# ipo-lab/lqp_py

Measured on AMD Instinct MI355X. Metric: QPs/sec forward+backward, batch=128 dz=500 tol=1e-5, higher is better.
Workload: dtype f32; 1 GPU; BASELINE configs[2]: batch=128/GPU dz=500 m=1 box+equality QP, ADMM forward + fixed-point backward, eps 1e-5, scale+adaptive_rho defaults; global_batch=128, seeds=10 batches, seeds 0..9 per rank, cycled, iters=60, checks=4, launch_mode=3, sync=False, linsolve=spd, loop_workgroups_per_qp=2, parallelism=batch-sharded x1, rccl_world_size=1

## Files before the change

lqp_py_amd/csrc/lqp_boxqp.hpp:

```cpp
#pragma once
#include <type_traits>
#include "lqp_common.hpp"
#include "lqp_lu.hpp"
#include "lqp_lu_big.hpp"
#include "lqp_lu2.hpp"
#include "lqp_lu_wide.hpp"
#include "lqp_trsv.hpp"
#include "lqp_spd.hpp"

namespace lqp {

enum { ST_DONE = 0, ST_FINAL_ITER = 1, ST_GATE = 2, ST_NFACTOR = 3, ST_RHO_UPDATED = 4,
       ST_TIMEOUT = 5, ST_NCHECK = 6, ST_NOTSPD = 7,
       ST_VOTE = 8,
       ST_ANY_LB = 12, ST_ANY_UB = 13,
       ST_RESUME = 14,
       ST_WORDS = 16 };
enum { RP_LB = 1, RP_UB = 2, RP_TIMEOUT = 4, RP_NOTSPD = 8 };
enum { CT_NOTOPT = 0, CT_ARRIVE = 1, CT_WANTS = 2, CT_TRIG = 3, CT_WORDS = 4 };
template <typename T>
__device__ __forceinline__ void trace_check(unsigned int* __restrict__ vtrace, const int it, const int check_solved, const int ring,
                                            const T pri, const T dua) {
    if (!vtrace) return;
    const int c = it / check_solved;
// ... 2351 lines not shown
        if (lane == 0) wtot[w] = __popcll(bal);
        __syncthreads();
        int base = nf;
#pragma unroll
        for (int ww = 0; ww < LQP_NW; ++ww) {
            const int c = wtot[ww];
            if (ww < w) base += c;
            nf += c;
        }
        if (keep) {
            fl[base + before] = i;
            if (blockIdx.y == 0) P.fidx[(size_t)b * n + base + before] = i;
        }
    }
    if (tid == 0 && blockIdx.y == 0) P.nred[b] = nf + m;
    __syncthreads();
    const int wy = blockIdx.y, ny = gridDim.y;
    constexpr int GQ = 8;
    for (int a0 = (w * ny + wy) * 2; a0 < nf; a0 += LQP_NW * ny * 2) {
        const int a1 = a0 + 1 < nf ? a0 + 1 : a0;
        const int i0 = fl[a0], i1 = fl[a1];
        const T* q0 = Q + (size_t)i0 * n;
        const T* q1 = Q + (size_t)i1 * n;
        const T dg0 = P.kkt ? kkt_weight(P, b, i0) : T(1e-8), dg1 = P.kkt ? kkt_weight(P, b, i1) : T(1e-8);
        for (int c0 = 0; c0 < nf; c0 += 64 * GQ) {
            T v0[GQ], v1[GQ];
#pragma unroll
            for (int q = 0; q < GQ; ++q) {
                const int c = c0 + lane + 64 * q;
                const int col = fl[c < nf ? c : nf - 1];
                v0[q] = q0[col];
                v1[q] = q1[col];
            }
#pragma unroll
            for (int q = 0; q < GQ; ++q) {
                const int c = c0 + lane + 64 * q;
                if (c < nf) {
                    M[(size_t)a0 * Np + c] = c == a0 ? v0[q] + dg0 : v0[q];
                    if (a1 != a0) M[(size_t)a1 * Np + c] = c == a1 ? v1[q] + dg1 : v1[q];
                }
            }
        }
        for (int r = lane; r < m; r += 64) {
            M[(size_t)a0 * Np + nf + r] = A[(size_t)r * n + i0];
            if (a1 != a0) M[(size_t)a1 * Np + nf + r] = A[(size_t)r * n + i1];
        }
        if (lane == 0 && P.g) { rhs[a0] = -g[i0]; if (a1 != a0) rhs[a1] = -g[i1]; }
    }
    for (int r = w * ny + wy; r < m; r += LQP_NW * ny) {
        T* mr = M + (size_t)(nf + r) * Np;
        for (int c = lane; c < nf; c += 64) mr[c] = A[(size_t)r * n + fl[c]];
        for (int c = lane; c < m; c += 64) mr[nf + c] = (c == r && !P.kkt) ? T(1e-8) : T(0);
        if (lane == 0) rhs[nf + r] = T(0);
    }
}

__device__ __forceinline__ float bwd_equil_scale(const float d) {
    if (!(d > 0.f) || !(d < 3.0e38f)) return 1.f;
    const int h = (int)((__float_as_uint(d) >> 23) & 0xFFu) - 127;
    return __uint_as_float((unsigned int)(127 - (h >> 1)) << 23);
}
template <int LQP_ANY = 0>
__global__ __launch_bounds__(LQP_NT) void k_bwd_build_chol(const BwdParams<float> P) {
    extern __shared__ __attribute__((aligned(32))) char smem[];
    const int b = blockIdx.x, n = P.n, m = P.m, Np = P.Np;
    const int tid = threadIdx.x, lane = tid & 63, w = tid >> 6;
    int* fl = (int*)smem;
    int* wtot = fl + round_up(n, 8);
    const float* x = P.x + (size_t)b * n;
    const float* u = P.u + (size_t)b * n;
    const float* lb = P.lb + (size_t)b * n;
    const float* ub = P.ub + (size_t)b * n;
    const float* g = P.g + (size_t)b * n;
    const float* Q = P.Q + (size_t)b * n * n;
    const float* A = P.A ? P.A + (size_t)b * m * n : nullptr;
    const int Kmax = round_up(n, LQP_NB) / LQP_NB, Npm = Kmax * LQP_NB;
    float* Ls = P.packed + (size_t)b * sym_blocks(Kmax) * LQP_BLK;
    float* AF = P.M + (size_t)b * Np * Np;
    float* rhs = P.rhs + (size_t)b * Np;
    if (tid == 0 && blockIdx.y == 0) P.info[b] = 0;
    float* wl = (float*)(wtot + LQP_NW + 8);
    bool keep = false;
    if (tid < n) {
        if (P.kkt) { keep = true; wl[tid] = kkt_weight(P, b, tid); }
        else {
            const float sxu = x[tid] + u[tid];
            keep = !(sxu > ub[tid] || sxu < lb[tid]);
        }
    }
    const unsigned long long bal = __ballot(keep);
    const int before = __popcll(bal & ((1ull << lane) - 1ull));
    if (lane == 0) wtot[w] = __popcll(bal);
    __syncthreads();
    int base = 0, nf = 0;
#pragma unroll
    for (int ww = 0; ww < LQP_NW; ++ww) {
        const int c = wtot[ww];
        if (ww < w) base += c;
        nf += c;
    }
    if (keep) {
        fl[base + before] = tid;
        if (blockIdx.y == 0) P.fidx[(size_t)b * n + base + before] = tid;
    }
    if (tid == 0 && blockIdx.y == 0) P.nred[b] = nf + m;
    __syncthreads();
    const int Kb = round_up(nf, LQP_NB) / LQP_NB;
    const int r = tid >> 4, c4 = (tid & 15) * 4;
    const int nblk = sym_blocks(Kb);
    float* const sl = wl + round_up(n, 8);
    for (int a = tid; a < Npm; a += LQP_NT) {
        float sv = 1.f;
        if (P.bsc && a < nf) sv = bwd_equil_scale(Q[(size_t)fl[a] * n + fl[a]] + (P.kkt ? wl[fl[a]] : 1e-8f));
        sl[a] = sv;
        if (P.bsc && blockIdx.y == 0) P.bsc[(size_t)b * Np + a] = sv;
    }
    __syncthreads();
    for (int t = blockIdx.y; t < nblk; t += gridDim.y) {
        int j = 0;
        while (sym_idx(j + 1, j + 1, Kb) <= t && j + 1 < Kb) ++j;
        const int i = j + (t - sym_idx(j, j, Kb));
        const int a = i * 64 + r;
        const bool rok = a < nf;
        const size_t rowoff = (size_t)fl[rok ? a : 0] * n;
        float q4[4];
#pragma unroll
        for (int e = 0; e < 4; ++e) {
            const int c = j * 64 + c4 + e;
            q4[e] = Q[rowoff + fl[c < nf ? c : 0]];
        }
        V4<float> v;
#pragma unroll
        for (int e = 0; e < 4; ++e) {
            const int c = j * 64 + c4 + e;
            float val = (a == c) ? 1.f : 0.f;
            if (rok && c < nf) val = ((q4[e] + (a == c ? (P.kkt ? wl[fl[a]] : 1e-8f) : 0.f)) * sl[a]) * sl[c];
            v.v[e] = val;
        }
        *(V4<float>*)(Ls + (size_t)t * LQP_BLK + tid * 4) = v;
    }
    if (blockIdx.y == 0) {
        if (P.phase != 1)
            for (int a = tid; a < Npm; a += LQP_NT) rhs[a] = a < nf ? -g[fl[a]] * sl[a] : 0.f;
        for (int q = 0; q < m; ++q)
            for (int a = tid; a < Npm; a += LQP_NT) AF[(size_t)q * Npm + a] = a < nf ? A[(size_t)q * n + fl[a]] * sl[a] : 0.f;
    }
}

__host__ __device__ inline int bwd_chol_lds_bytes(int n, int m, int nr = 2) {
    const int Kmax = round_up(n, LQP_NB) / LQP_NB, Npm = Kmax * LQP_NB;
    const int a0 = spd_lds_bytes(Kmax > SPD_MAXK ? SPD_MAXK : Kmax);
    const int a = (Kmax < SPD_MAXK && chol_la_lds_bytes(Kmax) > a0) ? chol_la_lds_bytes(Kmax) : a0;
    const int c = ((1 + nr + m) * Npm + nr * 64 + nr * LQP_NW * 64 + m * m + 2 * m + 8) * 4;
    return a > c ? a : c;
}
template <int NRV = 0, bool F16 = false>
__global__ __launch_bounds__(LQP_NT) void k_bwd_chol_solve(const BwdParams<float> P) {
    extern __shared__ __attribute__((aligned(32))) char smem[];
    const int b = blockIdx.x, n = P.n, m = P.m, Np = P.Np;
    const int tid = threadIdx.x, lane = tid & 63, w = tid >> 6;
    const int Kmax = round_up(n, LQP_NB) / LQP_NB, Npm = Kmax * LQP_NB;
    const int nf = P.nred[b] - m;
    const int Kb = round_up(nf, LQP_NB) / LQP_NB, Nb = Kb * LQP_NB;
    float* Ls = P.packed + (size_t)b * sym_blocks(Kmax) * LQP_BLK;
    const float* AF = P.M + (size_t)b * Np * Np;
    float* rhs = P.rhs + (size_t)b * Np;
    unsigned long long dt0 = P.dbg ? clock64() : 0;
    if (Kb > 0 && P.phase != 2) {
        if (Kb <= P.la_maxk) wg_chol_factor_la<F16>(Ls, Kb, P.info + b, smem, P.dbg ? P.dbg + (size_t)b * 8 : nullptr);
        else if (Kb <= SPD_MAXK) wg_chol_factor(Ls, Kb, P.info + b, smem);
        else wg_chol_factor_big(Ls, Kb, P.info + b, smem);
    }
    if (P.host_report && (P.early_report || P.phase == 1) && !P.reported) {
        __syncthreads();
        if (tid == 0)
            __hip_atomic_store(P.host_report + b, __hip_atomic_load(P.info + b, __ATOMIC_RELAXED, __HIP_MEMORY_SCOPE_AGENT),
                               __ATOMIC_RELAXED, __HIP_MEMORY_SCOPE_SYSTEM);
    }
    if (P.phase == 1) return;
    __syncthreads();
    if (P.dbg && tid == 0) { const unsigned long long t = clock64(); P.dbg[(size_t)b * 8 + 0] = t - dt0; dt0 = t; P.dbg[(size_t)b * 8 + 3] = Kb; }
    constexpr int NR = NRV == 4 ? 4 : 2;
    float* acc = (float*)smem;
    float* u0 = acc + (size_t)NR * Npm;
    float* G = u0 + Npm;
    float* t = G + (size_t)m * Npm;
    float* part = t + NR * 64;
    float* S = part + NR * LQP_NW * 64;
    float* wv = S + m * m;
    float* dn = wv + m;
    if (P.phase == 2) {
        const float* g = P.g + (size_t)b * n;
        const int* fidx = P.fidx + (size_t)b * n;
        const float* bs_ = P.bsc ? P.bsc + (size_t)b * Np : nullptr;
        for (int e = tid; e < Nb; e += LQP_NT) u0[e] = e < nf ? -g[fidx[e]] * (bs_ ? bs_[e] : 1.f) : 0.f;
    } else {
        for (int e = tid; e < Nb; e += LQP_NT) u0[e] = rhs[e];
    }
    for (int q = 0; q < m; ++q)
        for (int e = tid; e < Nb; e += LQP_NT) G[(size_t)q * Npm + e] = AF[(size_t)q * Npm + e];
    __syncthreads();
    if (Kb > 0)
        for (int c0 = 0; c0 < 1 + m; c0 += NR)
            wg_chol_solve_n<NR>(Ls, Kb, u0 + (size_t)c0 * Npm, Npm, (1 + m - c0) < NR ? (1 + m - c0) : NR, acc, t, part,
                                (P.dbg && P.la_maxk == 0) ? P.dbg + (size_t)b * 8 : nullptr);
    if (P.dbg && tid == 0) { const unsigned long long t = clock64(); P.dbg[(size_t)b * 8 + 1] = t - dt0; dt0 = t; }
    if (m > 0) {
        for (int e = w; e < m * m + m; e += LQP_NW) {
            const int q = e < m * m ? e / m : e - m * m;
            const float* rv = e < m * m ? G + (size_t)(e - q * m) * Npm : u0;
            float a = 0.f;
            for (int i = lane; i < nf; i += 64) a += AF[(size_t)q * Npm + i] * rv[i];
            a = wave_sum(a);
            if (lane == 0) {
                if (e < m * m) S[e] = a - ((e / m == e % m) ? 1e-8f : 0.f);
                else wv[q] = a;
            }
        }
        __syncthreads();
        {
            const int rr = tid / (m + 1), jj = tid - rr * (m + 1);
            const bool mine = tid < m * (m + 1);
            int* pivrow = (int*)dn;
            for (int c = 0; c < m; ++c) {
                if (tid == 0) {
                    int pr = c;
                    float best = tabs(S[c * m + c]);
                    for (int r2 = c + 1; r2 < m; ++r2) if (tabs(S[r2 * m + c]) > best) { best = tabs(S[r2 * m + c]); pr = r2; }
                    const bool skip = !(best > 0.f);
                    if (skip && P.info[b] == 0) P.info[b] = nf + c + 1;
                    pivrow[0] = pr; pivrow[1] = skip ? 1 : 0;
                }
                __syncthreads();
                const int pr = pivrow[0];
                const bool skip = pivrow[1] != 0;
                float* const rowc = jj < m ? S + c * m + jj : wv + c;
                float* const rowp = jj < m ? S + pr * m + jj : wv + pr;
                float* const rowr = jj < m ? S + rr * m + jj : wv + rr;
                if (!skip && pr != c && tid <= m) {
                    const float tmp = *rowc; *rowc = *rowp; *rowp = tmp;
                }
                __syncthreads();
                const float inv = skip ? 0.f : 1.f / S[c * m + c];
                const float f = (mine && !skip) ? S[rr * m + c] : 0.f;
                __syncthreads();
                if (!skip && tid <= m) *rowc *= inv;
                __syncthreads();
                if (mine && !skip && rr != c) *rowr -= f * *rowc;
                __syncthreads();
            }
            for (int q = tid; q < m; q += LQP_NT) dn[q] = wv[q];
        }
        __syncthreads();
    }
    for (int a = tid; a < nf; a += LQP_NT) {
        float d = u0[a];
        for (int q = 0; q < m; ++q) d -= G[(size_t)q * Npm + a] * dn[q];
        rhs[a] = P.bsc ? d * P.bsc[(size_t)b * Np + a] : d;
    }
    for (int q = tid; q < m; q += LQP_NT) rhs[nf + q] = dn[q];
    if (P.dbg && tid == 0) P.dbg[(size_t)b * 8 + 2] = clock64() - dt0;
}

template <typename T>
__global__ __launch_bounds__(LQP_NT) void k_bwd_residual(const BwdParams<T> P) {
    extern __shared__ __attribute__((aligned(32))) char smem[];
    const int b = blockIdx.x, n = P.n, m = P.m, Np = P.Np;
    const int tid = threadIdx.x, lane = tid & 63, w = tid >> 6;
    T* dvf = (T*)smem;
    T* dn = dvf + round_up(n, 8);
    int* fl = (int*)(dn + round_up(m > 0 ? m : 1, 8));
    const int nf = P.nred[b] - m;
    const T* d = P.rhs + (size_t)b * Np;
    T* r = P.rhs2 + (size_t)b * Np;
    const T* Q = P.Q + (size_t)b * n * n;
    const T* A = P.A ? P.A + (size_t)b * m * n : nullptr;
    const T* g = P.g + (size_t)b * n;
    for (int i = tid; i < n; i += LQP_NT) dvf[i] = T(0);
    for (int a = tid; a < nf; a += LQP_NT) fl[a] = P.fidx[(size_t)b * n + a];
    for (int q = tid; q < m; q += LQP_NT) dn[q] = d[nf + q];
    __syncthreads();
    for (int a = tid; a < nf; a += LQP_NT) dvf[fl[a]] = d[a];
    __syncthreads();
    constexpr int RG = 4;
    const int ny = (int)gridDim.y, me = (int)blockIdx.y;
    for (int a0 = (w * ny + me) * RG; a0 < nf + m; a0 += LQP_NW * ny * RG) {
        const T* row[RG];
        double acc[RG];
#pragma unroll
        for (int u = 0; u < RG; ++u) {
            const int a = min(a0 + u, nf + m - 1);
            row[u] = a >= nf ? A + (size_t)(a - nf) * n : Q + (size_t)fl[a] * n;
            acc[u] = 0.0;
        }
        for (int j = lane; j < n; j += 64) {
            const double dj = (double)dvf[j];
            T v[RG];
#pragma unroll
            for (int u = 0; u < RG; ++u) v[u] = row[u][j];
#pragma unroll
            for (int u = 0; u < RG; ++u) acc[u] += (double)v[u] * dj;
        }
#pragma unroll
        for (int u = 0; u < RG; ++u) acc[u] = wave_sum(acc[u]);
        if (lane < RG && a0 + lane < nf + m) {
            const int a = a0 + lane;
            double mine = readlane_t(acc[0], 0);
#pragma unroll
            for (int u = 1; u < RG; ++u) { const double t = readlane_t(acc[u], 0); mine = lane == u ? t : mine; }
            double res;
            if (a < nf) {
                const int i = fl[a];
                res = -(double)g[i] - mine - 1e-8 * (double)d[a];
                for (int q = 0; q < m; ++q) res -= (double)A[(size_t)q * n + i] * (double)dn[q];
            } else {
                res = -mine - 1e-8 * (double)dn[a - nf];
            }
            r[a] = (T)res;
        }
    }
    if (me == 0)
        for (int a = nf + m + tid; a < Np; a += LQP_NT) r[a] = T(0);
}

template <typename T> __host__ __device__ inline int solve_lds_bytes(int Np) { return (Np + 64) * (int)sizeof(T) + Np * 4; }

template <typename T>
__global__ __launch_bounds__(LQP_NT) void k_packed_solve(const T* __restrict__ packed_all, const int Nuni, const int Npmax,
                                                         const int Kmax, const int* __restrict__ dest_all,
                                                         T* __restrict__ rhs_all, const int nrhs,
                                                         const size_t rhs_bstride, const int rhs_rstride,
                                                         const int rhs_cstride, const int* __restrict__ Nvec) {
    extern __shared__ __attribute__((aligned(32))) char smem[];
    const int b = blockIdx.x, tid = threadIdx.x;
    const int N = Nvec ? Nvec[b] : Nuni;
    const int K = round_up(N, LQP_NB) / LQP_NB, Np = K * LQP_NB;
    T* v = (T*)smem;
    T* tmp = v + Npmax;
    int* dest = (int*)(tmp + 64);
    const T* packed = packed_all + (size_t)b * packed_blocks(Kmax) * LQP_BLK;
    const int S = K * (K + 1);
    const bool cyclic = true;
    BlockStream<T, LQP_NT> st;
    stream_prime(st, packed, S);
    for (int i = tid; i < Np; i += LQP_NT) dest[i] = dest_all[(size_t)b * Npmax + i];
    __syncthreads();
    T* rhs = rhs_all + (size_t)b * rhs_bstride;
    for (int c = 0; c < nrhs; ++c) {
        for (int i = tid; i < Np; i += LQP_NT) v[dest[i]] = (i < N) ? rhs[(size_t)i * rhs_rstride + (size_t)c * rhs_cstride] : T(0);
        wg_barrier_lds();
        wg_packed_solve(st, packed, K, v, tmp, cyclic && (c + 1 < nrhs));
        if (!cyclic && c + 1 < nrhs) stream_prime(st, packed, S);
        for (int i = tid; i < N; i += LQP_NT) rhs[(size_t)i * rhs_rstride + (size_t)c * rhs_cstride] = v[i];
        __syncthreads();
    }
}

template <typename T>
__global__ __launch_bounds__(LQP_NT) void k_bwd_epilogue(const BwdParams<T> P) {
    extern __shared__ __attribute__((aligned(32))) char smem[];
    const int b = blockIdx.x, n = P.n, m = P.m, Np = P.Np;
    const int tid = threadIdx.x, lane = tid & 63, w = tid >> 6;
    T* dv = (T*)smem;
    T* xs = dv + n;
    T* dnu = xs + n;
    const T rho = (P.rho_mode == 2) ? P.rho_in[b] : P.rho_value;
    const T* d = P.rhs + (size_t)b * Np;
    const T* x = P.x + (size_t)b * n;
    const T poison = P.info[b] != 0 ? T(__builtin_nanf("")) : T(0);
    if (P.host_report && !(P.chol && P.early_report) && !P.lu_reported && tid == 0 && blockIdx.y == 0)
        __hip_atomic_store(P.host_report + b, P.info[b], __ATOMIC_RELAXED, __HIP_MEMORY_SCOPE_SYSTEM);
    if (P.reduced) {
        const int nf = P.nred[b] - m;
        const int* fl = P.fidx + (size_t)b * n;
        const T* d2 = P.rhs2 + (size_t)b * Np;
        for (int i = tid; i < n; i += LQP_NT) { dv[i] = poison; xs[i] = x[i]; }
        __syncthreads();
        for (int a = tid; a < nf; a += LQP_NT) dv[fl[a]] = d[a] + (P.refine ? d2[a] : T(0)) + poison;
        for (int r = tid; r < m; r += LQP_NT) dnu[r] = d[nf + r] + (P.refine ? d2[nf + r] : T(0)) + poison;
    } else {
        for (int i = tid; i < n; i += LQP_NT) { dv[i] = d[i] + poison; xs[i] = x[i]; }
        for (int r = tid; r < m; r += LQP_NT) dnu[r] = d[n + r] + poison;
    }
    __syncthreads();
    const bool first = blockIdx.y == 0;
    if (P.dp && first) for (int i = tid; i < n; i += LQP_NT) P.dp[(size_t)b * n + i] = dv[i];
    if (P.db && first) for (int r = tid; r < m; r += LQP_NT) P.db[(size_t)b * m + r] = -dnu[r];
    if (P.dA && m > 0 && first) {
        const T* nus = P.nus + (size_t)b * m;
        for (int t = tid; t < m * n; t += LQP_NT) {
            const int r = t / n, j = t - r * n;
            P.dA[(size_t)b * m * n + t] = dnu[r] * xs[j] + nus[r] * dv[j];
        }
    }
    const T* Q = P.Q + (size_t)b * n * n;
    const T* A = P.A ? P.A + (size_t)b * m * n : nullptr;
    if (P.kkt && first) {
        for (int i = tid; i < n; i += LQP_NT) {
            const T xi = xs[i];
            const T slo = tmax(xi - P.lb[(size_t)b * n + i], T(1e-8)), shi = tmax(P.ub[(size_t)b * n + i] - xi, T(1e-8));
            const T llo = tmax(P.lams[(size_t)b * 2 * n + i], T(1e-8)), lhi = tmax(P.lams[(size_t)b * 2 * n + n + i], T(1e-8));
            if (P.dlb) P.dlb[(size_t)b * n + i] = llo * (-dv[i] / slo);
            if (P.dub) P.dub[(size_t)b * n + i] = -lhi * (dv[i] / shi);
        }
    }
    const bool need_kkt = (P.dlb || P.dub) && !P.kkt;
    T* dQ = P.dQ ? P.dQ + (size_t)b * n * n : nullptr;
    const bool vec = (n % 4 == 0) && n <= 1024 && dQ && ((((uintptr_t)dQ) % sizeof(V4<T>)) == 0);
    V4<T> xj[4], hj[4];
    if (vec) {
// ... 136 lines not shown
```

lqp_py_amd/csrc/lqp_spd.hpp:

```cpp
#pragma once
#include "lqp_common.hpp"
#include "lqp_lu.hpp"
#include "lqp_trsv.hpp"
#include "lqp_f16x2.hpp"

namespace lqp {

constexpr int SPD_LS = 68;
constexpr int SPD_MAXK = 8;
constexpr int SPD_MAXM = 16;

__host__ __device__ constexpr int sym_blocks(int K) { return K * (K + 1) / 2; }
__host__ __device__ constexpr int sym_idx(int i, int j, int K) { return j * K - j * (j - 1) / 2 + (i - j); }
#ifndef LQP_PIV_WAVES
#define LQP_PIV_WAVES 16
#endif
#ifndef LQP_PIV_WAVES_RS
#define LQP_PIV_WAVES_RS 8
#endif
#ifndef LQP_PIV_NB
#define LQP_PIV_NB 4
#endif
constexpr int PIV_NB = LQP_PIV_NB;
constexpr int PIV_LDS = 2 * PIV_NB * 64 + 64;
// ... 2500 lines not shown
                int si = 0;
                while ((si + 1) * (si + 2) / 2 <= p) ++si;
                const int sj = p - si * (si + 1) / 2;
                if (si == sj && qi == 0 && qj == 1) continue;
                float* T0 = Hs + (size_t)sym_idx(k + 1 + si, k + 1 + sj, K) * LQP_BLK;
                float* C = T0 + (32 * qi) * 64 + 32 * qj + li;
                f32x16 cur;
#pragma unroll
                for (int q = 0; q < 16; ++q) cur[q] = C[quad_row(q, lh) * 64];
                const f32x16 acc = spd_quadrant(Y + ((size_t)si * 64 + 32 * qi) * SPD_LS,
                                                Y + ((size_t)sj * 64 + 32 * qj) * SPD_LS);
                cur -= acc;
#pragma unroll
                for (int q = 0; q < 16; ++q) C[quad_row(q, lh) * 64] = cur[q];
                if (si == sj && qi == 1 && qj == 0) {
#pragma unroll
                    for (int q = 0; q < 16; ++q) T0[li * 64 + 32 + quad_row(q, lh)] = cur[q];
                }
            }
        }
        __syncthreads();
    }
    if (tid == 0 && flag[0] != 0 && *info == 0) *info = flag[0];
}

__device__ __forceinline__ void wg_chol_factor_big(float* __restrict__ Hs, const int K, int* __restrict__ info, char* smem) {
    constexpr int CH = SPD_MAXK - 1;
    const int tid = threadIdx.x, lane = tid & 63, w = tid >> 6;
    const int r = tid >> 4, cq = tid & 15, li = lane & 31, lh = lane >> 5;
    float* Y = (float*)smem;
    float* W = Y + (size_t)CH * 64 * SPD_LS;
    float* WT = W + 64 * SPD_LS;
    float* pcol = WT + 64 * SPD_LS;
    int* flag = (int*)(pcol + PIV_LDS);
    if (tid == 0) flag[0] = 0;
    for (int k = 0; k < K; ++k) {
        const int np = K - 1 - k;
        wg_pivot<LQP_PIV_WAVES>(Hs + (size_t)sym_idx(k, k, K) * LQP_BLK, W, WT, pcol, flag, k * 64);
        __syncthreads();
        *(V4<float>*)(Hs + (size_t)sym_idx(k, k, K) * LQP_BLK + tid * 4) = *(const V4<float>*)(W + r * SPD_LS + cq * 4);
        for (int c0 = 0; c0 < np; c0 += CH) {
            const int cn = (np - c0) < CH ? (np - c0) : CH;
            for (int u = 0; u < cn; ++u)
                *(V4<float>*)(Y + ((size_t)u * 64 + r) * SPD_LS + cq * 4) =
                    *(const V4<float>*)(Hs + (size_t)sym_idx(k + 1 + c0 + u, k, K) * LQP_BLK + tid * 4);
            __syncthreads();
            {
                const int ntask = cn * 4;
                f32x16 acc[2];
#pragma unroll
                for (int u = 0; u < 2; ++u) {
                    const int task = __builtin_amdgcn_readfirstlane(w + 16 * u);
                    if (task < ntask) {
                        const int sl = task >> 2, qi = (task >> 1) & 1, qj = task & 1;
                        const float* Xp = Y + ((size_t)sl * 64 + 32 * qi) * SPD_LS;
                        acc[u] = qj == 0 ? spd_quadrant<1, false>(Xp, W) : spd_quadrant(Xp, W + 32 * SPD_LS);
                    }
                }
                __syncthreads();
#pragma unroll
                for (int u = 0; u < 2; ++u) {
                    const int task = __builtin_amdgcn_readfirstlane(w + 16 * u);
                    if (task < ntask) {
                        const int sl = task >> 2, qi = (task >> 1) & 1, qj = task & 1;
                        float* dst = Y + ((size_t)sl * 64 + 32 * qi) * SPD_LS + 32 * qj + li;
#pragma unroll
                        for (int q = 0; q < 16; ++q) dst[quad_row(q, lh) * SPD_LS] = acc[u][q];
                    }
                }
                __syncthreads();
            }
            for (int u = 0; u < cn; ++u)
                *(V4<float>*)(Hs + (size_t)sym_idx(k + 1 + c0 + u, k, K) * LQP_BLK + tid * 4) =
                    *(const V4<float>*)(Y + ((size_t)u * 64 + r) * SPD_LS + cq * 4);
            __syncthreads();
        }
        __threadfence_block();
        __syncthreads();
        const int ng = (np + BIG_G - 1) / BIG_G;
        for (int ga = 0; ga < ng; ++ga) {
            for (int gb = 0; gb <= ga; ++gb) {
                const int a0 = BIG_G * ga, b0 = BIG_G * gb;
                const int an = (np - a0) < BIG_G ? (np - a0) : BIG_G, bn = (np - b0) < BIG_G ? (np - b0) : BIG_G;
                const int boff = gb == ga ? 0 : BIG_G;
                for (int u = 0; u < an; ++u)
                    *(V4<float>*)(Y + ((size_t)u * 64 + r) * SPD_LS + cq * 4) =
                        *(const V4<float>*)(Hs + (size_t)sym_idx(k + 1 + a0 + u, k, K) * LQP_BLK + tid * 4);
                if (gb != ga)
                    for (int u = 0; u < bn; ++u)
                        *(V4<float>*)(Y + ((size_t)(BIG_G + u) * 64 + r) * SPD_LS + cq * 4) =
                            *(const V4<float>*)(Hs + (size_t)sym_idx(k + 1 + b0 + u, k, K) * LQP_BLK + tid * 4);
                __syncthreads();
                const int npair = gb == ga ? an * (an + 1) / 2 : an * bn;
                auto decode = [&](const int task, int& ua, int& ub, bool& skip, bool& mirror) -> float* {
                    const int qi = (task >> 1) & 1, qj = task & 1, p = task >> 2;
                    if (gb == ga) {
                        ua = 0;
                        while ((ua + 1) * (ua + 2) / 2 <= p) ++ua;
                        ub = p - ua * (ua + 1) / 2;
                    } else {
                        ua = p / bn;
                        ub = p - ua * bn;
                    }
                    const int si = a0 + ua, sj = b0 + ub;
                    skip = si == sj && qi == 0 && qj == 1;
                    mirror = si == sj && qi == 1 && qj == 0;
                    return Hs + (size_t)sym_idx(k + 1 + si, k + 1 + sj, K) * LQP_BLK;
                };
                auto load_c = [&](const float* T0, const int task, f32x16& c) {
                    const float* C = T0 + (32 * ((task >> 1) & 1)) * 64 + 32 * (task & 1) + li;
#pragma unroll
                    for (int q = 0; q < 16; ++q) c[q] = C[quad_row(q, lh) * 64];
                };
                const int ntask = npair * 4;
                int task = __builtin_amdgcn_readfirstlane(w);
                int ua = 0, ub = 0; bool skip = false, mirror = false;
                float* T0 = nullptr;
                f32x16 nxt;
                if (task < ntask) { T0 = decode(task, ua, ub, skip, mirror); if (!skip) load_c(T0, task, nxt); }
                while (task < ntask) {
                    const int qi = (task >> 1) & 1, qj = task & 1;
                    f32x16 cur = nxt;
                    float* Tc = T0;
                    const int cua = ua, cub = ub;
                    const bool cskip = skip, cmirror = mirror;
                    const int nt = task + LQP_NW;
                    if (nt < ntask) { T0 = decode(nt, ua, ub, skip, mirror); if (!skip) load_c(T0, nt, nxt); }
                    if (!cskip) {
                        const f32x16 acc = spd_quadrant(Y + ((size_t)cua * 64 + 32 * qi) * SPD_LS,
                                                        Y + ((size_t)(boff + cub) * 64 + 32 * qj) * SPD_LS);
                        cur -= acc;
                        float* C = Tc + (32 * qi) * 64 + 32 * qj + li;
#pragma unroll
                        for (int q = 0; q < 16; ++q) C[quad_row(q, lh) * 64] = cur[q];
                        if (cmirror) {
#pragma unroll
                            for (int q = 0; q < 16; ++q) Tc[li * 64 + 32 + quad_row(q, lh)] = cur[q];
                        }
                    }
                    task = nt;
                }
                __syncthreads();
            }
        }
        __threadfence_block();
        __syncthreads();
    }
    if (tid == 0 && flag[0] != 0 && *info == 0) *info = flag[0];
}

constexpr int CHOL_LA_CHAIN = 4;
__host__ __device__ inline int chol_la_lds_bytes(int K) { return spd_lds_bytes(K) + 64 + 64 * 64 * 4; }

template <bool F16 = false>
__device__ __forceinline__ void wg_chol_factor_la(float* __restrict__ Hs, const int K, int* __restrict__ info, char* smem,
                                                  unsigned long long* __restrict__ dbg = nullptr) {
    constexpr int NCH = CHOL_LA_CHAIN, NTW = LQP_NW - NCH, NTT = NTW * 64;
    const int tid = threadIdx.x, lane = tid & 63, w = tid >> 6;
    const int li = lane & 31, lh = lane >> 5;
    const int nslot = K > 1 ? K - 1 : 1;
    float* Y = (float*)smem;
    float* W = Y + (size_t)nslot * 64 * SPD_LS;
    float* WT = W + 64 * SPD_LS;
    float* pcol = WT + 64 * SPD_LS;
    int* flag = (int*)(pcol + PIV_LDS);
    int* sy = flag + 4;
    float* St = (float*)(flag + 20);
    if (tid < 20) flag[tid] = 0;
    *(V4<float>*)(St + tid * 4) = *(const V4<float>*)(Hs + (size_t)sym_idx(0, 0, K) * LQP_BLK + tid * 4);
    __syncthreads();
    if (w < NCH) {
        __builtin_amdgcn_s_setprio(3);
        int gt = 0;
        for (int k = 0; k < K; ++k) {
            unsigned long long c0 = dbg ? clock64() : 0;
            lds_wait_ge(sy + 2, 3 * k);
            lds_wait_ge(sy + 4, k);
            if (dbg && tid == 0) { const unsigned long long c1 = clock64(); dbg[4] += c1 - c0; c0 = c1; }
#if LQP_PIV_MFMA
            wg_pivot_block_mfma<true, true, false, F16>(St, W, WT, pcol, flag, k * 64, sy + 5, k, 0.f, false, pcol + 128);
#else
            wg_pivot_block<NCH, true>(St, W, WT, pcol, flag, k * 64, sy + 0, &gt);
#endif
            lds_group_sync<true>(sy + 0, gt += NCH);
            if (tid == 0) __hip_atomic_store(sy + 3, k + 1, __ATOMIC_RELAXED, __HIP_MEMORY_SCOPE_WORKGROUP);
            for (int v = tid; v < 1024; v += NCH * 64)
                *(V4<float>*)(Hs + (size_t)sym_idx(k, k, K) * LQP_BLK + v * 4) = *(const V4<float>*)(W + (v >> 4) * SPD_LS + (v & 15) * 4);
            if (dbg && tid == 0) dbg[5] += clock64() - c0;
        }
        __builtin_amdgcn_s_setprio(0);
    } else {
        const int tw = w - NCH, tt = tid - NCH * 64;
        int gt = 0;
        for (int k = 0; k < K; ++k) {
            const int np = K - 1 - k;
            for (int s = 0; s < np; ++s) {
                const float* src = Hs + (size_t)sym_idx(k + 1 + s, k, K) * LQP_BLK;
                for (int v = tt; v < 1024; v += NTT)
                    *(V4<float>*)(Y + ((size_t)s * 64 + (v >> 4)) * SPD_LS + (v & 15) * 4) = *(const V4<float>*)(src + v * 4);
            }
            const int nupd = np * (np + 1) / 2 * 4;
            f32x16 pre;
            if (tw < nupd && !(tw == 1)) {
                const int qi = (tw >> 1) & 1, qj = tw & 1, p = tw >> 2;
                int si = 0;
                while ((si + 1) * (si + 2) / 2 <= p) ++si;
                const int sj = p - si * (si + 1) / 2;
                if (!(si == sj && qi == 0 && qj == 1)) {
                    const float* C = Hs + (size_t)sym_idx(k + 1 + si, k + 1 + sj, K) * LQP_BLK + (32 * qi) * 64 + 32 * qj + li;
#pragma unroll
                    for (int q = 0; q < 16; ++q) pre[q] = C[quad_row(q, lh) * 64];
                }
            }
            lds_group_sync(sy + 1, gt += NTW);
            unsigned long long c0 = dbg ? clock64() : 0;
            lds_wait_ge(sy + 3, k + 1);
            if (dbg && tt == 0) { const unsigned long long c1 = clock64(); dbg[6] += c1 - c0; c0 = c1; }
            [[maybe_unused]] float* const ysc = pcol + 144;
            [[maybe_unused]] char* const Yc = (char*)Y;
            [[maybe_unused]] const int lane_b = li * F2_ROW + 32 * lh;
            if constexpr (F16) {
                float sW, isW;
                f2_scale_of(tmax((pcol + 128)[1], (pcol + 128)[2]), sW, isW);
                for (int task = tw; task < np * 2; task += NTW) {
                    const int s = task >> 1, qi = task & 1;
                    const float* prow = Y + ((size_t)s * 64 + 32 * qi + li) * SPD_LS;
                    float pv[4][8], mx = 0.f;
#pragma unroll
                    for (int c = 0; c < 4; ++c) {
                        f2_load_cell_f32(prow, c, lh, pv[c]);
#pragma unroll
                        for (int j = 0; j < 8; ++j) mx = tmax(mx, tabs(pv[c][j]));
                    }
                    mx = wave_max(mx);
                    float sP, isP;
                    f2_scale_of(mx, sP, isP);
                    F2Cell pb[4];
#pragma unroll
                    for (int c = 0; c < 4; ++c) {
#pragma unroll
                        for (int j = 0; j < 8; ++j) pv[c][j] *= sP;
                        f2_split8(pv[c], pb[c].hi, pb[c].mid);
                    }
                    f32x16 a0, a1;
#pragma unroll
                    for (int q = 0; q < 16; ++q) { a0[q] = 0.f; a1[q] = 0.f; }
#pragma unroll
                    for (int c = 0; c < 4; ++c) {
                        float wv[8];
                        F2Cell wc;
                        if (c < 2) {
                            f2_load_cell_f32(W + li * SPD_LS, c, lh, wv);
#pragma unroll
                            for (int j = 0; j < 8; ++j) wv[j] *= sW;
                            f2_split8(wv, wc.hi, wc.mid);
                            a0 = f2_mma(wc, pb[c], a0);
                        }
                        f2_load_cell_f32(W + (32 + li) * SPD_LS, c, lh, wv);
#pragma unroll
                        for (int j = 0; j < 8; ++j) wv[j] *= sW;
                        f2_split8(wv, wc.hi, wc.mid);
                        a1 = f2_mma(wc, pb[c], a1);
                    }
                    const float un = isW * isP;
                    if (lane == 0) ysc[task] = un * 2097152.f;
                    float* dstg = Hs + (size_t)sym_idx(k + 1 + s, k, K) * LQP_BLK + (32 * qi + li) * 64 + 4 * lh;
                    char* dstl = Yc + ((size_t)s * 64 + 32 * qi) * F2_ROW + lane_b;
#pragma unroll
                    for (int hsel = 0; hsel < 2; ++hsel) {
#pragma unroll
                        for (int c = 0; c < 2; ++c) {
                            float v[8];
#pragma unroll
                            for (int gq = 0; gq < 2; ++gq) {
                                V4<float> o;
#pragma unroll
                                for (int e = 0; e < 4; ++e) {
                                    const float a = hsel ? a1[8 * c + 4 * gq + e] : a0[8 * c + 4 * gq + e];
                                    o.v[e] = a * un;
                                    v[4 * gq + e] = a * 4.76837158203125e-7f;
                                }
                                *(V4<float>*)(dstg + 32 * hsel + 8 * (2 * c + gq)) = o;
                            }
                            h16x8 hi, mid;
                            f2_split8(v, hi, mid);
                            f2_write_cell(dstl + 64 * (2 * hsel + c), hi, mid);
                        }
                    }
                }
            } else {
            for (int task = tw; task < np * 2; task += NTW) {
                const int s = task >> 1, qi = task & 1;
                float* Xp = Y + ((size_t)s * 64 + 32 * qi) * SPD_LS;
                const f32x16 a0 = spd_quadrant<1, false>(Xp, W);
                const f32x16 a1 = spd_quadrant(Xp, W + 32 * SPD_LS);
#pragma unroll
                for (int q = 0; q < 16; ++q) {
                    Xp[quad_row(q, lh) * SPD_LS + li] = a0[q];
                    Xp[quad_row(q, lh) * SPD_LS + 32 + li] = a1[q];
                }
            }
            }
            lds_group_sync(sy + 1, gt += NTW);
            if (tt == 0) __hip_atomic_store(sy + 4, k + 1, __ATOMIC_RELEASE, __HIP_MEMORY_SCOPE_WORKGROUP);
            {
                for (int task = tw; task < nupd; task += NTW) {
                    const int qi = (task >> 1) & 1, qj = task & 1, p = task >> 2;
                    int si = 0;
                    while ((si + 1) * (si + 2) / 2 <= p) ++si;
                    const int sj = p - si * (si + 1) / 2;
                    if (si == sj && qi == 0 && qj == 1) continue;
                    float* T0 = Hs + (size_t)sym_idx(k + 1 + si, k + 1 + sj, K) * LQP_BLK;
                    float* C = T0 + (32 * qi) * 64 + 32 * qj + li;
                    f32x16 cur;
                    if (task == tw) cur = pre;
                    else {
#pragma unroll
                        for (int q = 0; q < 16; ++q) cur[q] = C[quad_row(q, lh) * 64];
                    }
                    if constexpr (F16) {
                        const f32x16 acc = f2_quadrant<0, 4>(Yc + ((size_t)si * 64 + 32 * qi) * F2_ROW + lane_b,
                                                             Yc + ((size_t)sj * 64 + 32 * qj) * F2_ROW + lane_b);
                        const float un = -(ysc[2 * si + qi] * ysc[2 * sj + qj]);
#pragma unroll
                        for (int q = 0; q < 16; ++q) cur[q] = __builtin_fmaf(acc[q], un, cur[q]);
                    } else {
                    const f32x16 acc = spd_quadrant(Y + ((size_t)si * 64 + 32 * qi) * SPD_LS,
                                                    Y + ((size_t)sj * 64 + 32 * qj) * SPD_LS);
                    cur -= acc;
                    }
                    if (p == 0) {
                        float* Sq = St + (32 * qi) * 64 + 32 * qj + li;
#pragma unroll
                        for (int q = 0; q < 16; ++q) Sq[quad_row(q, lh) * 64] = cur[q];
                        if (qi == 1 && qj == 0) {
#pragma unroll
                            for (int q = 0; q < 16; ++q) St[li * 64 + 32 + quad_row(q, lh)] = cur[q];
                        }
                        asm volatile("s_waitcnt lgkmcnt(0)" ::: "memory");
                        if (lane == 0) __hip_atomic_fetch_add(sy + 2, 1, __ATOMIC_RELAXED, __HIP_MEMORY_SCOPE_WORKGROUP);
                    }
#pragma unroll
                    for (int q = 0; q < 16; ++q) C[quad_row(q, lh) * 64] = cur[q];
                    if (si == sj && qi == 1 && qj == 0) {
#pragma unroll
                        for (int q = 0; q < 16; ++q) T0[li * 64 + 32 + quad_row(q, lh)] = cur[q];
                    }
                }
                if constexpr (!F16) {
                for (int s = 0; s < np; ++s) {
                    float* dst = Hs + (size_t)sym_idx(k + 1 + s, k, K) * LQP_BLK;
                    for (int v = tt; v < 1024; v += NTT)
                        *(V4<float>*)(dst + v * 4) = *(const V4<float>*)(Y + ((size_t)s * 64 + (v >> 4)) * SPD_LS + (v & 15) * 4);
                }
                }
            }
            lds_group_sync(sy + 1, gt += NTW);
            if (dbg && tt == 0) dbg[7] += clock64() - c0;
        }
    }
    __syncthreads();
    if (tid == 0 && flag[0] != 0 && *info == 0) *info = flag[0];
}

template <int NR>
__device__ __forceinline__ void wg_chol_solve_n(const float* __restrict__ Ls, const int K, float* __restrict__ X, const int xs,
                                                const int nc, float* __restrict__ acc, float* __restrict__ t,
                                                float* __restrict__ part, unsigned long long* __restrict__ dbg = nullptr) {
    constexpr int MC = SPD_MAXK - 1;
    unsigned long long c0 = dbg ? clock64() : 0;
    const int tid = threadIdx.x, r = tid >> 4, cq = tid & 15, lane = tid & 63, w = tid >> 6;
    const int K64 = K * 64;
    const int tc = tid >> 6, te = tid & 63;
    auto blk4 = [&](const int i, const int j) -> V4<float> {
        return *(const V4<float>*)(Ls + (size_t)sym_idx(i, j, K) * LQP_BLK + tid * 4);
    };
    for (int e = tid; e < NR * K64; e += LQP_NT) acc[e] = 0.f;
    V4<float> bd = blk4(0, 0);
    __syncthreads();
    for (int j = 0; j < K; ++j) {
        V4<float> bc[MC];
#pragma unroll
        for (int u = 0; u < MC; ++u)
            if (j + 1 + u < K) bc[u] = blk4(j + 1 + u, j);
        if (tc < nc) t[tc * 64 + te] = X[(size_t)tc * xs + j * 64 + te] - acc[tc * K64 + j * 64 + te];
        __syncthreads();
#pragma unroll
        for (int c = 0; c < NR; ++c) {
            if (c < nc) {
                const float s1 = rowgroup_sum<LQP_NT>(dot4(bd, *(const V4<float>*)(t + c * 64 + cq * 4)));
                if (cq == 0) X[(size_t)c * xs + j * 64 + r] = s1;
            }
        }
        if (j + 1 < K) bd = blk4(j + 1, j + 1);
        __syncthreads();
        V4<float> yj[NR];
#pragma unroll
        for (int c = 0; c < NR; ++c) yj[c] = *(const V4<float>*)(X + (size_t)(c < nc ? c : 0) * xs + j * 64 + cq * 4);
        for (int u0 = 0; j + 1 + u0 < K; u0 += MC) {
            if (u0 > 0) {
#pragma unroll
                for (int u = 0; u < MC; ++u)
                    if (j + 1 + u0 + u < K) bc[u] = blk4(j + 1 + u0 + u, j);
            }
#pragma unroll
            for (int u = 0; u < MC; ++u) {
                const int i = j + 1 + u0 + u;
                if (i < K) {
#pragma unroll
                    for (int c = 0; c < NR; ++c) {
                        if (c < nc) {
                            const float s1 = rowgroup_sum<LQP_NT>(dot4(bc[u], yj[c]));
                            if (cq == 0) acc[c * K64 + i * 64 + r] += s1;
                        }
                    }
                }
            }
        }
        __syncthreads();
    }
    auto fold = [&](float (&a2)[4], const int c) {
        col_fold<4>(a2);
        part[((size_t)c * LQP_NW + w) * 64 + cq * 4 + col_fold_elem(lane)] = a2[0];
    };
    if (dbg && threadIdx.x == 0) { const unsigned long long c1 = clock64(); dbg[4] += c1 - c0; c0 = c1; }
    bd = blk4(K - 1, K - 1);
    for (int j = K - 1; j >= 0; --j) {
        V4<float> bc[MC];
#pragma unroll
        for (int u = 0; u < MC; ++u)
            if (j + 1 + u < K) bc[u] = blk4(j + 1 + u, j);
        float a2[NR][4];
#pragma unroll
        for (int c = 0; c < NR; ++c)
#pragma unroll
            for (int e = 0; e < 4; ++e) a2[c][e] = 0.f;
        for (int u0 = 0; j + 1 + u0 < K; u0 += MC) {
            if (u0 > 0) {
#pragma unroll
                for (int u = 0; u < MC; ++u)
                    if (j + 1 + u0 + u < K) bc[u] = blk4(j + 1 + u0 + u, j);
            }
#pragma unroll
            for (int u = 0; u < MC; ++u) {
                const int i = j + 1 + u0 + u;
                if (i < K) {
#pragma unroll
                    for (int c = 0; c < NR; ++c) {
                        const float xi = X[(size_t)(c < nc ? c : 0) * xs + i * 64 + r];
#pragma unroll
                        for (int e = 0; e < 4; ++e) a2[c][e] += bc[u].v[e] * xi;
                    }
                }
            }
        }
#pragma unroll
        for (int c = 0; c < NR; ++c) fold(a2[c], c);
        __syncthreads();
        if (tc < nc) {
            float sum = 0.f;
#pragma unroll
            for (int ww = 0; ww < LQP_NW; ++ww) sum += part[((size_t)tc * LQP_NW + ww) * 64 + te];
            t[tc * 64 + te] = X[(size_t)tc * xs + j * 64 + te] - sum;
        }
        __syncthreads();
#pragma unroll
        for (int c = 0; c < NR; ++c) {
            const float tr = t[c * 64 + r];
#pragma unroll
            for (int e = 0; e < 4; ++e) a2[c][e] = bd.v[e] * tr;
            fold(a2[c], c);
        }
        if (j > 0) bd = blk4(j - 1, j - 1);
        __syncthreads();
        if (tc < nc) {
            float sum = 0.f;
#pragma unroll
            for (int ww = 0; ww < LQP_NW; ++ww) sum += part[((size_t)tc * LQP_NW + ww) * 64 + te];
            X[(size_t)tc * xs + j * 64 + te] = sum;
        }
        __syncthreads();
    }
    if (dbg && threadIdx.x == 0) dbg[5] += clock64() - c0;
}

}
```

Measured before the change: 200,000 QPs/sec.

## Fuse forward triangular solve into look-ahead Cholesky factorization in backward kernel

In the backward Cholesky solve kernel, when m<=2 and the look-ahead factor path is used with F16, the forward substitution for the RHS and the constraint columns is folded into the factorization loop. After each diagonal block is factored, the triangular-solve updates run on LDS-resident copies, and the later solve skips its forward sweep. For m==1 the dense pivoted elimination of the small Schur system is replaced by a scalar division. It raises the LDS budget (capped at 160KB), which may reduce occupancy, and adds work to the chain waves inside the factor pipeline.

Measured after the change: 202,700 QPs/sec (median of 5 runs). +1.3%, better.

```diff
diff --git a/lqp_py_amd/csrc/lqp_boxqp.hpp b/lqp_py_amd/csrc/lqp_boxqp.hpp
--- a/lqp_py_amd/csrc/lqp_boxqp.hpp
+++ b/lqp_py_amd/csrc/lqp_boxqp.hpp
@@ -2527,7 +2527,13 @@
     const int a0 = spd_lds_bytes(Kmax > SPD_MAXK ? SPD_MAXK : Kmax);
     const int a = (Kmax < SPD_MAXK && chol_la_lds_bytes(Kmax) > a0) ? chol_la_lds_bytes(Kmax) : a0;
     const int c = ((1 + nr + m) * Npm + nr * 64 + nr * LQP_NW * 64 + m * m + 2 * m + 8) * 4;
-    return a > c ? a : c;
+    int r = a > c ? a : c;
+    if (nr == 2 && m <= 2) {
+        const int Kla = Kmax < SPD_MAXK ? Kmax : SPD_MAXK - 1;
+        const int f = chol_la_lds_bytes(Kla) + chol_fold_lds_bytes(Kla, 1 + m, m);
+        if (f <= 160 * 1024 && f > r) r = f;
+    }
+    return r;
 }
 template <int NRV = 0, bool F16 = false>
 __global__ __launch_bounds__(LQP_NT) void k_bwd_chol_solve(const BwdParams<float> P) {
@@ -2541,7 +2547,27 @@
     const float* AF = P.M + (size_t)b * Np * Np;
     float* rhs = P.rhs + (size_t)b * Np;
     unsigned long long dt0 = P.dbg ? clock64() : 0;
-    if (Kb > 0 && P.phase != 2) {
+    constexpr bool FOLD = LQP_BWD_FOLD && NRV == 0 && F16;
+    bool fold = false;
+    [[maybe_unused]] float* fX = nullptr;
+    [[maybe_unused]] float* fAF = nullptr;
+    if constexpr (FOLD) {
+        fold = P.phase == 0 && m <= 2 && Kb > 0 && Kb <= P.la_maxk &&
+               chol_la_lds_bytes(Kb) + chol_fold_lds_bytes(Kb, 1 + m, m) <= bwd_chol_lds_bytes(n, m, 2);
+        if (fold) {
+            fX = (float*)(smem + chol_la_lds_bytes(Kb));
+            float* const fAcc = fX + (size_t)(1 + m) * Nb;
+            float* const fT = fAcc + (size_t)(1 + m) * Nb;
+            fAF = fT + (1 + m) * 64;
+            for (int e = tid; e < Nb; e += LQP_NT) fX[e] = rhs[e];
+            for (int q = 0; q < m; ++q)
+                for (int e = tid; e < Nb; e += LQP_NT) { const float v = AF[(size_t)q * Npm + e]; fX[(size_t)(1 + q) * Nb + e] = v; fAF[(size_t)q * Nb + e] = v; }
+            for (int e = tid; e < (1 + m) * Nb; e += LQP_NT) fAcc[e] = 0.f;
+            wg_chol_factor_la<F16, true>(Ls, Kb, P.info + b, smem, P.dbg ? P.dbg + (size_t)b * 8 : nullptr, fX, Nb, 1 + m, fAcc, fT);
+        }
+    }
+    if (fold) {
+    } else if (Kb > 0 && P.phase != 2) {
         if (Kb <= P.la_maxk) wg_chol_factor_la<F16>(Ls, Kb, P.info + b, smem, P.dbg ? P.dbg + (size_t)b * 8 : nullptr);
         else if (Kb <= SPD_MAXK) wg_chol_factor(Ls, Kb, P.info + b, smem);
         else wg_chol_factor_big(Ls, Kb, P.info + b, smem);
@@ -2560,11 +2586,14 @@
     float* u0 = acc + (size_t)NR * Npm;
     float* G = u0 + Npm;
     float* t = G + (size_t)m * Npm;
+    const int xs = fold ? Nb : Npm;
+    if (fold) { u0 = fX; G = fX + Nb; }
     float* part = t + NR * 64;
     float* S = part + NR * LQP_NW * 64;
     float* wv = S + m * m;
     float* dn = wv + m;
-    if (P.phase == 2) {
+    if (fold) {
+    } else if (P.phase == 2) {
         const float* g = P.g + (size_t)b * n;
         const int* fidx = P.fidx + (size_t)b * n;
         const float* bs_ = P.bsc ? P.bsc + (size_t)b * Np : nullptr;
@@ -2572,20 +2601,22 @@
     } else {
         for (int e = tid; e < Nb; e += LQP_NT) u0[e] = rhs[e];
     }
-    for (int q = 0; q < m; ++q)
-        for (int e = tid; e < Nb; e += LQP_NT) G[(size_t)q * Npm + e] = AF[(size_t)q * Npm + e];
+    if (!fold)
+        for (int q = 0; q < m; ++q)
+            for (int e = tid; e < Nb; e += LQP_NT) G[(size_t)q * Npm + e] = AF[(size_t)q * Npm + e];
     __syncthreads();
     if (Kb > 0)
         for (int c0 = 0; c0 < 1 + m; c0 += NR)
-            wg_chol_solve_n<NR>(Ls, Kb, u0 + (size_t)c0 * Npm, Npm, (1 + m - c0) < NR ? (1 + m - c0) : NR, acc, t, part,
-                                (P.dbg && P.la_maxk == 0) ? P.dbg + (size_t)b * 8 : nullptr);
+            wg_chol_solve_n<NR, FOLD>(Ls, Kb, u0 + (size_t)c0 * xs, xs, (1 + m - c0) < NR ? (1 + m - c0) : NR, acc, t, part,
+                                (P.dbg && P.la_maxk == 0) ? P.dbg + (size_t)b * 8 : nullptr, fold);
     if (P.dbg && tid == 0) { const unsigned long long t = clock64(); P.dbg[(size_t)b * 8 + 1] = t - dt0; dt0 = t; }
     if (m > 0) {
         for (int e = w; e < m * m + m; e += LQP_NW) {
             const int q = e < m * m ? e / m : e - m * m;
-            const float* rv = e < m * m ? G + (size_t)(e - q * m) * Npm : u0;
+            const float* rv = e < m * m ? G + (size_t)(e - q * m) * xs : u0;
+            const float* av = fold ? fAF + (size_t)q * Nb : AF + (size_t)q * Npm;
             float a = 0.f;
-            for (int i = lane; i < nf; i += 64) a += AF[(size_t)q * Npm + i] * rv[i];
+            for (int i = lane; i < nf; i += 64) a += av[i] * rv[i];
             a = wave_sum(a);
             if (lane == 0) {
                 if (e < m * m) S[e] = a - ((e / m == e % m) ? 1e-8f : 0.f);
@@ -2593,7 +2624,14 @@
             }
         }
         __syncthreads();
-        {
+        if (fold && m == 1) {
+            if (tid == 0) {
+                const float s0 = S[0];
+                const bool skip = !(tabs(s0) > 0.f);
+                if (skip && P.info[b] == 0) P.info[b] = nf + 1;
+                dn[0] = skip ? wv[0] : wv[0] * (1.f / s0);
+            }
+        } else {
             const int rr = tid / (m + 1), jj = tid - rr * (m + 1);
             const bool mine = tid < m * (m + 1);
             int* pivrow = (int*)dn;
@@ -2630,7 +2668,7 @@
     }
     for (int a = tid; a < nf; a += LQP_NT) {
         float d = u0[a];
-        for (int q = 0; q < m; ++q) d -= G[(size_t)q * Npm + a] * dn[q];
+        for (int q = 0; q < m; ++q) d -= G[(size_t)q * xs + a] * dn[q];
         rhs[a] = P.bsc ? d * P.bsc[(size_t)b * Np + a] : d;
     }
     for (int q = tid; q < m; q += LQP_NT) rhs[nf + q] = dn[q];
diff --git a/lqp_py_amd/csrc/lqp_spd.hpp b/lqp_py_amd/csrc/lqp_spd.hpp
--- a/lqp_py_amd/csrc/lqp_spd.hpp
+++ b/lqp_py_amd/csrc/lqp_spd.hpp
@@ -2676,9 +2676,17 @@
 constexpr int CHOL_LA_CHAIN = 4;
 __host__ __device__ inline int chol_la_lds_bytes(int K) { return spd_lds_bytes(K) + 64 + 64 * 64 * 4; }
 
-template <bool F16 = false>
+#ifndef LQP_BWD_FOLD
+#define LQP_BWD_FOLD 1
+#endif
+__host__ __device__ inline int chol_fold_lds_bytes(int K, int nc, int m) { return ((2 * nc + m) * K * 64 + nc * 64) * 4; }
+
+template <bool F16 = false, bool FOLD = false>
 __device__ __forceinline__ void wg_chol_factor_la(float* __restrict__ Hs, const int K, int* __restrict__ info, char* smem,
-                                                  unsigned long long* __restrict__ dbg = nullptr) {
+                                                  unsigned long long* __restrict__ dbg = nullptr,
+                                                  [[maybe_unused]] float* __restrict__ fx = nullptr, [[maybe_unused]] const int fxs = 0,
+                                                  [[maybe_unused]] const int fnc = 0, [[maybe_unused]] float* __restrict__ facc = nullptr,
+                                                  [[maybe_unused]] float* __restrict__ ft = nullptr) {
     constexpr int NCH = CHOL_LA_CHAIN, NTW = LQP_NW - NCH, NTT = NTW * 64;
     const int tid = threadIdx.x, lane = tid & 63, w = tid >> 6;
     const int li = lane & 31, lh = lane >> 5;
@@ -2711,6 +2719,62 @@
             for (int v = tid; v < 1024; v += NCH * 64)
                 *(V4<float>*)(Hs + (size_t)sym_idx(k, k, K) * LQP_BLK + v * 4) = *(const V4<float>*)(W + (v >> 4) * SPD_LS + (v & 15) * 4);
             if (dbg && tid == 0) dbg[5] += clock64() - c0;
+            if constexpr (FOLD) {
+                if (fx) {
+                    const unsigned long long f0 = dbg ? clock64() : 0;
+                    constexpr int FNC = 3;
+                    const int fr = tid >> 4, fq = (tid & 15) * 4;
+                    auto apply = [&](const int j, const int i0, const int i1) {
+                        V4<float> yj[FNC];
+#pragma unroll
+                        for (int c = 0; c < FNC; ++c) yj[c] = *(const V4<float>*)(fx + (size_t)(c < fnc ? c : 0) * fxs + j * 64 + fq);
+                        for (int i = i0; i < i1; i += 2) {
+                            V4<float> bl[2][4];
+#pragma unroll
+                            for (int u = 0; u < 2; ++u) {
+                                const float* src = Hs + (size_t)sym_idx(i + u < i1 ? i + u : i, j, K) * LQP_BLK + tid * 4;
+#pragma unroll
+                                for (int p = 0; p < 4; ++p) bl[u][p] = *(const V4<float>*)(src + p * 1024);
+                            }
+#pragma unroll
+                            for (int u = 0; u < 2; ++u) {
+                                if (i + u < i1) {
+#pragma unroll
+                                    for (int c = 0; c < FNC; ++c) {
+                                        if (c < fnc) {
+#pragma unroll
+                                            for (int p = 0; p < 4; ++p) {
+                                                const float s1 = rowgroup_sum<LQP_NT>(dot4(bl[u][p], yj[c]));
+                                                if (fq == 0) facc[(size_t)c * fxs + (i + u) * 64 + 16 * p + fr] += s1;
+                                            }
+                                        }
+                                    }
+                                }
+                            }
+                        }
+                    };
+                    if (k > 0) apply(k - 1, k + 1, K);
+                    if (tid < fnc * 64) ft[tid] = fx[(size_t)w * fxs + k * 64 + lane] - facc[(size_t)w * fxs + k * 64 + lane];
+                    lds_group_sync<true>(sy + 0, gt += NCH);
+#pragma unroll
+                    for (int c = 0; c < FNC; ++c) {
+                        if (c < fnc) {
+#pragma unroll
+                            for (int p = 0; p < 4; ++p) {
+                                const float s1 = rowgroup_sum<LQP_NT>(dot4(*(const V4<float>*)(W + (16 * p + fr) * SPD_LS + fq),
+                                                                          *(const V4<float>*)(ft + c * 64 + fq)));
+                                if (fq == 0) fx[(size_t)c * fxs + k * 64 + 16 * p + fr] = s1;
+                            }
+                        }
+                    }
+                    lds_group_sync<true>(sy + 0, gt += NCH);
+                    if (k + 1 < K) {
+                        lds_wait_ge(sy + 4, k + 1);
+                        apply(k, k + 1, k + 2);
+                    }
+                    if (dbg && tid == 0) dbg[4] += (clock64() - f0) << 32;
+                }
+            }
         }
         __builtin_amdgcn_s_setprio(0);
     } else {
@@ -2887,10 +2951,12 @@
     if (tid == 0 && flag[0] != 0 && *info == 0) *info = flag[0];
 }
 
-template <int NR>
+template <int NR, bool MAY_HAVE_Y = false>
 __device__ __forceinline__ void wg_chol_solve_n(const float* __restrict__ Ls, const int K, float* __restrict__ X, const int xs,
                                                 const int nc, float* __restrict__ acc, float* __restrict__ t,
-                                                float* __restrict__ part, unsigned long long* __restrict__ dbg = nullptr) {
+                                                float* __restrict__ part, unsigned long long* __restrict__ dbg = nullptr,
+                                                const bool have_y_in = false) {
+    const bool have_y = MAY_HAVE_Y && have_y_in;
     constexpr int MC = SPD_MAXK - 1;
     unsigned long long c0 = dbg ? clock64() : 0;
     const int tid = threadIdx.x, r = tid >> 4, cq = tid & 15, lane = tid & 63, w = tid >> 6;
@@ -2899,10 +2965,10 @@
     auto blk4 = [&](const int i, const int j) -> V4<float> {
         return *(const V4<float>*)(Ls + (size_t)sym_idx(i, j, K) * LQP_BLK + tid * 4);
     };
-    for (int e = tid; e < NR * K64; e += LQP_NT) acc[e] = 0.f;
-    V4<float> bd = blk4(0, 0);
+    if (!have_y) for (int e = tid; e < NR * K64; e += LQP_NT) acc[e] = 0.f;
+    V4<float> bd = blk4(have_y ? K - 1 : 0, have_y ? K - 1 : 0);
     __syncthreads();
-    for (int j = 0; j < K; ++j) {
+    for (int j = have_y ? K : 0; j < K; ++j) {
         V4<float> bc[MC];
 #pragma unroll
         for (int u = 0; u < MC; ++u)
@@ -2948,7 +3014,7 @@
         part[((size_t)c * LQP_NW + w) * 64 + cq * 4 + col_fold_elem(lane)] = a2[0];
     };
     if (dbg && threadIdx.x == 0) { const unsigned long long c1 = clock64(); dbg[4] += c1 - c0; c0 = c1; }
-    bd = blk4(K - 1, K - 1);
+    if (!have_y) bd = blk4(K - 1, K - 1);
     for (int j = K - 1; j >= 0; --j) {
         V4<float> bc[MC];
 #pragma unroll
```
